# ViacheslavDanilov/oct_segmentation

Measured on AMD Instinct MI355X. Metric: OCT frames/sec (704x704, bf16) fwd+bwd, higher is better.
Workload: dtype bf16; 1 GPU; unetplusplus/resnet101 1-class 704x704, batch 16/GPU, fwd+Dice+bwd+allreduce+Adam; global_batch=16, parallelism=dp1

## Files before the change

oct_segmentation_amd/csrc/wgrad_mfma.hip:

```cpp
#include "common.h"
#include "conv_common.h"
#include "kernels.h"

#include <cstdlib>
#include <type_traits>

namespace octseg {

#ifdef OCTSEG_STAMP
#define WSTAMP(var) do { __builtin_amdgcn_sched_barrier(0); asm volatile("s_memtime %0\n\ts_waitcnt lgkmcnt(0)" : "=s"(var) :: "memory"); __builtin_amdgcn_sched_barrier(0); } while (0)
#else
#define WSTAMP(var) do { } while (0)
#endif

typedef __attribute__((ext_vector_type(4))) short s16x4_t;
typedef __attribute__((address_space(3))) s16x4_t lds_s16x4_t;

template <int NTAPS> struct WgradCfg { static constexpr int MAXW = NTAPS == 1 ? 4 : (NTAPS == 4 ? 6 : 7); };

__host__ __device__ constexpr int wrow_slots_before(int wr, int ks, int th) {
  int n = 0;
  for (int w = 0; w < wr; ++w) {
    const int klo = w - (ks - 1) < 0 ? 0 : w - (ks - 1), khi = w < th ? w : th - 1;
    n += (khi - klo + 1) * ks;
  }
  return n;
}

template <typename T, int NTAPS>
__global__ __launch_bounds__(NTHR) void wgrad_mfma_kernel(const WgradArgs a, const int th, const int pipelined) {
  extern __shared__ __attribute__((aligned(16))) char smem[];
  constexpr int VEC = Tr<T>::VEC;
  constexpr int RB = 64 * (int)sizeof(T);
  constexpr int PITCH = sizeof(T) == 2 ? 192 : RB + 16;
  constexpr int VPR = RB / 16;
  constexpr int PSTEP = NTHR / VPR;
  constexpr int MAXY = 4, MAXW = WgradCfg<NTAPS>::MAXW;
  typedef WindowStager<T, RB, NTHR, PITCH> Stager;

  const int tid = threadIdx.x, lane = tid & 63, wave = tid >> 6;
  const int wq_m = wave >> 1, wq_n = wave & 1;
  int bx = blockIdx.x, by = blockIdx.y, bz = blockIdx.z;
  {
    const int gx_ = gridDim.x, gy_ = gridDim.y, gz_ = gridDim.z;
    const int total = gx_ * gy_ * gz_;
    const int groups = gx_ * gz_;
    const int lid = bx + gx_ * (by + gy_ * bz);
    if (a.co_fast && (groups & 7) == 0) {
      const int x = lid & 7, q = lid >> 3;
      const int k = q / gy_, r = q - k * gy_;
      const int g = x * (groups >> 3) + k;
      by = r; bz = g / gx_; bx = g - bz * gx_;
    } else if (!a.co_fast && (total & 7) == 0 && (gz_ & 7) == 0) {
      const int w = (lid & 7) * (total >> 3) + (lid >> 3);
      bz = w / (gx_ * gy_);
      const int rem = w - bz * (gx_ * gy_);
      by = rem / gx_; bx = rem - by * gx_;
    }
  }
  const int ci0 = bx * 64, co0 = by * 64;

  const int tiles_x = (a.OW + TW - 1) / TW, tiles_y = (a.OH + th - 1) / th;
  const int ntiles = a.N * tiles_x * tiles_y;

  const bool single = a.ntaps == 1;
  const int lstride = single ? 1 : a.istride;
  const int smul = single ? a.istride : 1;
  const int RH = single ? th : (th - 1) * a.istride + a.span_y;
  const int RW = single ? TW : (TW - 1) * a.istride + a.span_x;
  const int npix = RH * RW;
  const int npw = (npix + PSTEP - 1) / PSTEP;
  const int npy = (th * TW + PSTEP - 1) / PSTEP;
  const float inv_rw = 1.0f / (float)RW;

  char* ldsY = smem;
  char* ldsX = smem + npy * PSTEP * PITCH;

  f32x16_t acc[NTAPS];
#pragma unroll
  for (int t = 0; t < NTAPS; ++t)
#pragma unroll
    for (int k = 0; k < 16; ++k) acc[t][k] = 0.f;

  int toff[NTAPS];
#pragma unroll
  for (int t = 0; t < NTAPS; ++t)
    toff[t] = single ? 0 : ((a.tap_dy[t] - a.min_dy) * RW + (a.tap_dx[t] - a.min_dx)) * PITCH;

  int ya0, xa0, xrow_step;
  if constexpr (sizeof(T) == 2) {
    const int g = lane >> 4, i = lane & 15, q = i >> 2, p = i & 3, hh = g >> 1, cb = g & 1;
    const int tx = 8 * hh + q;
    ya0 = tx * PITCH + (wq_m * 32 + 16 * cb + 4 * p) * 2;
    xa0 = (tx * lstride) * PITCH + (wq_n * 32 + 16 * cb + 4 * p) * 2;
    xrow_step = 4 * lstride * PITCH;
  } else {
    const int r = lane & 31, h = lane >> 5;
    ya0 = h * PITCH + (wq_m * 32 + r) * 4;
    xa0 = (h * lstride) * PITCH + (wq_n * 32 + r) * 4;
    xrow_step = 2 * lstride * PITCH;
  }

  Stager sg;
  sg.setup(a.src, a.nsrc, a.Cin, bx, tid);
  const int ycv = tid % VPR, yp0 = tid / VPR;
  const int yc = co0 + ycv * VEC;
  const bool ycok = yc < a.dyC;

  struct TilePos { int n, y0, x0; };
  auto tile_pos = [&](int tile) {
    TilePos tp;
    tp.n = tile / (tiles_x * tiles_y);
    const int rem = tile - tp.n * tiles_x * tiles_y;
    const int tyi = rem / tiles_x;
    tp.y0 = tyi * th; tp.x0 = (rem - tyi * tiles_x) * TW;
    return tp;
  };
  const int dy_pix_bytes = a.dyC * (int)sizeof(T), dy_row_bytes = a.DW * dy_pix_bytes;
  auto load_y = [&](const char* ybase, const TilePos& tp, int ty, int tx, bool in_tile, bool& ok) {
    const int gy = tp.y0 + ty, gx = tp.x0 + tx;
    ok = ycok && in_tile && gy < a.OH && gx < a.OW;
    const int gyc = min(gy, a.OH - 1), gxc = min(gx, a.OW - 1);
    const unsigned off = (unsigned)((gyc * a.dstride + a.doy) * dy_row_bytes + (gxc * a.dstride + a.dox) * dy_pix_bytes);
    return *(const uint4*)(ybase + off);
  };
  auto write_y = [&](int pass, uint4 v, bool ok) {
    *(uint4*)(ldsY + (pass * PSTEP + yp0) * PITCH + ycv * 16) = ok ? v : make_uint4(0, 0, 0, 0);
  };
  auto y_base = [&](int n) { return (const char*)a.dy + ((size_t)n * a.DH * a.DW * a.dyC + (ycok ? yc : 0)) * sizeof(T); };
  auto compute = [&]() {
    if constexpr (sizeof(T) == 2) {
      struct Pair { s16x4_t lo, hi; };
      struct Frags { uint4 y; uint4 x[NTAPS]; };
      auto load_frags = [&](int kk, Frags& f) {
        const char* yrow = ldsY + kk * TW * PITCH + ya0;
        const char* xrow = ldsX + (kk * lstride) * RW * PITCH + xa0;
        Pair ya;
        ya.lo = __builtin_amdgcn_ds_read_tr16_b64_v4i16((lds_s16x4_t*)(yrow));
        ya.hi = __builtin_amdgcn_ds_read_tr16_b64_v4i16((lds_s16x4_t*)(yrow + 4 * PITCH));
        f.y = __builtin_bit_cast(uint4, ya);
#pragma unroll
        for (int t = 0; t < NTAPS; ++t) {
          Pair xb;
          xb.lo = __builtin_amdgcn_ds_read_tr16_b64_v4i16((lds_s16x4_t*)(xrow + toff[t]));
          xb.hi = __builtin_amdgcn_ds_read_tr16_b64_v4i16((lds_s16x4_t*)(xrow + toff[t] + xrow_step));
          f.x[t] = __builtin_bit_cast(uint4, xb);
        }
      };
      auto load_y1 = [&](int kk, Frags& f) {
        const char* yrow = ldsY + kk * TW * PITCH + ya0;
        Pair ya;
        ya.lo = __builtin_amdgcn_ds_read_tr16_b64_v4i16((lds_s16x4_t*)(yrow));
        ya.hi = __builtin_amdgcn_ds_read_tr16_b64_v4i16((lds_s16x4_t*)(yrow + 4 * PITCH));
        f.y = __builtin_bit_cast(uint4, ya);
      };
      auto load_x1 = [&](const char* xrow, int t, Frags& f) {
        Pair xb;
        xb.lo = __builtin_amdgcn_ds_read_tr16_b64_v4i16((lds_s16x4_t*)(xrow + toff[t]));
        xb.hi = __builtin_amdgcn_ds_read_tr16_b64_v4i16((lds_s16x4_t*)(xrow + toff[t] + xrow_step));
        f.x[t] = __builtin_bit_cast(uint4, xb);
      };
      auto row_step = [&](const Frags& cur, int kn, Frags& nxt) {
        const char* xrow = ldsX + (kn * lstride) * RW * PITCH + xa0;
#pragma unroll
        for (int t = 0; t < NTAPS; ++t) {
          Tr<T>::mma(cur.y, cur.x[t], acc[t]);
          __builtin_amdgcn_sched_barrier(0);
          if (t == 0) load_y1(kn, nxt);
          load_x1(xrow, t, nxt);
          __builtin_amdgcn_sched_barrier(0);
        }
      };
      Frags fa, fb;
      load_frags(0, fa);
      for (int kk = 0; kk < th; kk += 2) {
        row_step(fa, min(kk + 1, th - 1), fb);
        if (kk + 1 < th) row_step(fb, min(kk + 2, th - 1), fa);
      }
    } else {
      for (int kk = 0; kk < th; ++kk) {
        const char* yrow = ldsY + kk * TW * PITCH + ya0;
        const char* xrow = ldsX + (kk * lstride) * RW * PITCH + xa0;
#pragma unroll
        for (int kp = 0; kp < 8; ++kp) {
          const float yv = *(const float*)(yrow + kp * 2 * PITCH);
#pragma unroll
          for (int t = 0; t < NTAPS; ++t) {
            const float xv = *(const float*)(xrow + toff[t] + kp * xrow_step);
            acc[t] = __builtin_amdgcn_mfma_f32_32x32x2f32(yv, xv, acc[t], 0, 0, 0);
          }
        }
      }
    }
  };

#ifdef OCTSEG_STAMP
  unsigned long long wts[5] = {0, 0, 0, 0, 0};
#endif
  if (pipelined) {
    uint4 yv[MAXY], xv[MAXW];
    bool yok[MAXY], xok[MAXW];
    int ypos[MAXY], wpos[MAXW];
    bool yin[MAXY], win[MAXW];
#pragma unroll
    for (int u = 0; u < MAXY; ++u) {
      const int p = min(u, npy - 1) * PSTEP + yp0;
      ypos[u] = ((p >> 4) << 16) | (p & 15);
      yin[u] = p < th * TW;
    }
#pragma unroll
    for (int u = 0; u < MAXW; ++u) {
      const int hp = min(u, npw - 1) * PSTEP + sg.p0;
      const int hy = (int)(((float)hp + 0.5f) * inv_rw);
      wpos[u] = (hy << 16) | (hp - hy * RW);
      win[u] = hp < npix;
    }
    auto load_tile = [&](int tile) {
      const TilePos tp = tile_pos(tile);
      const char* yb = y_base(tp.n);
      sg.bind_image(tp.n);
      const int gy0 = tp.y0 * a.istride + a.min_dy, gx0 = tp.x0 * a.istride + a.min_dx;
#pragma unroll
      for (int u = 0; u < MAXY; ++u) yv[u] = load_y(yb, tp, ypos[u] >> 16, ypos[u] & 0xffff, yin[u], yok[u]);
#pragma unroll
      for (int u = 0; u < MAXW; ++u)
        xv[u] = sg.load_at(wpos[u] >> 16, wpos[u] & 0xffff, win[u], gy0, gx0, smul, a.IH, a.IW, xok[u]);
    };
    auto write_tile = [&]() {
#pragma unroll
      for (int u = 0; u < MAXY; ++u) write_y(min(u, npy - 1), yv[u], yok[u]);
#pragma unroll
      for (int u = 0; u < MAXW; ++u) sg.write(ldsX, min(u, npw - 1), xv[u], xok[u]);
    };
    int tile = bz;
    if constexpr (sizeof(T) == 2 && (NTAPS == 9 || NTAPS == 4)) {
      if (pipelined == 2 && tile < ntiles) {
        constexpr int TH8 = 8, NSLOT = TH8 * NTAPS, NITEM = MAXY + MAXW, KS = NTAPS == 9 ? 3 : 2, RWC = TW + KS - 1, NWR = TH8 + KS - 1;
        const int tile_bytes = (npy + npw) * PSTEP * PITCH;
        TilePos tp2{0, 0, 0};
        const char* yb2 = nullptr;
        int gy02 = 0, gx02 = 0;
        auto item = [&](auto jc, auto phase, char* oy, char* ox) __attribute__((always_inline)) {
          constexpr int J = decltype(jc)::value;
          constexpr int PH = decltype(phase)::value;
          if constexpr (PH == 0) {
            if constexpr (J < MAXY) *(uint4*)(oy + (min(J, npy - 1) * PSTEP + yp0) * PITCH + ycv * 16) = yok[J] ? yv[J] : make_uint4(0, 0, 0, 0);
            else sg.write(ox, min(J - MAXY, npw - 1), xv[J - MAXY], xok[J - MAXY]);
          } else {
            if constexpr (J < MAXY) yv[J] = load_y(yb2, tp2, ypos[J] >> 16, ypos[J] & 0xffff, yin[J], yok[J]);
            else xv[J - MAXY] = sg.load_at(wpos[J - MAXY] >> 16, wpos[J - MAXY] & 0xffff, win[J - MAXY], gy02, gx02, smul, a.IH, a.IW, xok[J - MAXY]);
          }
        };
        auto fillers = [&](auto sc_, char* oy, char* ox) __attribute__((always_inline)) {
          constexpr int S = decltype(sc_)::value;
          constexpr int HALF = NSLOT / 2;
          constexpr int PH = S < HALF ? 0 : 1;
          constexpr int SS = S - PH * HALF;
          constexpr int J0 = (SS * NITEM + HALF - 1) / HALF, J1 = ((SS + 1) * NITEM + HALF - 1) / HALF;
          if constexpr (J0 < J1 && J0 < NITEM) item(std::integral_constant<int, J0>{}, std::integral_constant<int, PH>{}, oy, ox);
          if constexpr (J0 + 1 < J1 && J0 + 1 < NITEM) item(std::integral_constant<int, J0 + 1>{}, std::integral_constant<int, PH>{}, oy, ox);
          if constexpr (J0 + 2 < J1 && J0 + 2 < NITEM) item(std::integral_constant<int, J0 + 2>{}, std::integral_constant<int, PH>{}, oy, ox);
        };
        struct Frag { s16x4_t lo, hi; };
        Frag xs[2][KS], ys[4];
        auto rd_x = [&](const char* xbase, auto wc, auto sc, auto hc) __attribute__((always_inline)) {
          constexpr int Wn = decltype(wc)::value, S_ = decltype(sc)::value, H_ = decltype(hc)::value;
          constexpr int OFF = (Wn * RWC + S_) * PITCH + H_ * 4 * PITCH;
          if constexpr (H_ == 0) xs[Wn & 1][S_].lo = __builtin_amdgcn_ds_read_tr16_b64_v4i16((lds_s16x4_t*)(xbase + OFF));
          else xs[Wn & 1][S_].hi = __builtin_amdgcn_ds_read_tr16_b64_v4i16((lds_s16x4_t*)(xbase + OFF));
        };
        auto rd_y = [&](const char* ybase, auto kc, auto hc) __attribute__((always_inline)) {
          constexpr int Kn = decltype(kc)::value, H_ = decltype(hc)::value;
          constexpr int OFF = Kn * TW * PITCH + H_ * 4 * PITCH;
          if constexpr (H_ == 0) ys[Kn & 3].lo = __builtin_amdgcn_ds_read_tr16_b64_v4i16((lds_s16x4_t*)(ybase + OFF));
          else ys[Kn & 3].hi = __builtin_amdgcn_ds_read_tr16_b64_v4i16((lds_s16x4_t*)(ybase + OFF));
        };
        auto prefetch = [&](auto wc, auto qc, const char* xbase, const char* ybase) __attribute__((always_inline)) {
          constexpr int Q = decltype(qc)::value;
          if constexpr (Q < 2 * KS) rd_x(xbase, wc, std::integral_constant<int, Q / 2>{}, std::integral_constant<int, Q % 2>{});
          else rd_y(ybase, wc, std::integral_constant<int, Q - 2 * KS>{});
        };
        auto wrow = [&](auto wc, const char* by, const char* bx, char* oy, char* ox) __attribute__((always_inline)) {
          constexpr int Wr = decltype(wc)::value;
          constexpr int KLO = Wr - (KS - 1) < 0 ? 0 : Wr - (KS - 1), KHI = Wr < TH8 ? Wr : TH8 - 1;
          constexpr int CNT = (KHI - KLO + 1) * KS;
          constexpr int S0 = wrow_slots_before(Wr, KS, TH8);
          constexpr int NR = Wr + 1 >= NWR ? 0 : (Wr + 1 < TH8 ? 2 * KS + 2 : 2 * KS);
          const char* xbase = bx + xa0;
          const char* ybase = by + ya0;
          auto one = [&](auto jc) __attribute__((always_inline)) {
            constexpr int j = decltype(jc)::value;
            if constexpr (j < CNT) {
              constexpr int kk = KLO + j / KS, sft = j % KS, t = NTAPS == 9 ? (Wr - kk) * 3 + sft : (1 - (Wr - kk)) * 2 + (1 - sft);
              Tr<T>::mma(__builtin_bit_cast(uint4, ys[kk & 3]), __builtin_bit_cast(uint4, xs[Wr & 1][sft]), acc[t]);
              __builtin_amdgcn_sched_barrier(0);
              constexpr int R0 = j * NR / CNT, R1 = (j + 1) * NR / CNT;
              if constexpr (R0 < R1) prefetch(std::integral_constant<int, Wr + 1>{}, std::integral_constant<int, R0>{}, xbase, ybase);
              if constexpr (R0 + 1 < R1) prefetch(std::integral_constant<int, Wr + 1>{}, std::integral_constant<int, R0 + 1>{}, xbase, ybase);
              if constexpr (R0 + 2 < R1) prefetch(std::integral_constant<int, Wr + 1>{}, std::integral_constant<int, R0 + 2>{}, xbase, ybase);
              fillers(std::integral_constant<int, S0 + j>{}, oy, ox);
              __builtin_amdgcn_sched_barrier(0);
            }
          };
          one(std::integral_constant<int, 0>{}); one(std::integral_constant<int, 1>{}); one(std::integral_constant<int, 2>{});
          one(std::integral_constant<int, 3>{}); one(std::integral_constant<int, 4>{}); one(std::integral_constant<int, 5>{});
          one(std::integral_constant<int, 6>{}); one(std::integral_constant<int, 7>{}); one(std::integral_constant<int, 8>{});
        };
        load_tile(tile);
        write_tile();
        load_tile(tile + a.ksplit < ntiles ? tile + a.ksplit : tile);
        __syncthreads();
        int cur = 0;
        for (; tile < ntiles; tile += a.ksplit) {
          const int t2 = tile + 2 * a.ksplit < ntiles ? tile + 2 * a.ksplit : tile;
          tp2 = tile_pos(t2);
          yb2 = y_base(tp2.n);
          gy02 = tp2.y0 * a.istride + a.min_dy; gx02 = tp2.x0 * a.istride + a.min_dx;
          const char* by = smem + cur * tile_bytes;
          const char* bx = by + npy * PSTEP * PITCH;
          char* oy = smem + (cur ^ 1) * tile_bytes;
          char* ox = oy + npy * PSTEP * PITCH;
          {
            auto z = std::integral_constant<int, 0>{};
            auto o = std::integral_constant<int, 1>{};
            rd_y(by + ya0, z, z); rd_y(by + ya0, z, o);
            rd_x(bx + xa0, z, z, z); rd_x(bx + xa0, z, z, o);
            rd_x(bx + xa0, z, o, z); rd_x(bx + xa0, z, o, o);
            if constexpr (KS == 3) { rd_x(bx + xa0, z, std::integral_constant<int, 2>{}, z); rd_x(bx + xa0, z, std::integral_constant<int, 2>{}, o); }
          }
          wrow(std::integral_constant<int, 0>{}, by, bx, oy, ox);
          wrow(std::integral_constant<int, 1>{}, by, bx, oy, ox);
          wrow(std::integral_constant<int, 2>{}, by, bx, oy, ox);
          wrow(std::integral_constant<int, 3>{}, by, bx, oy, ox);
          if constexpr (KS == 2) sg.bind_image(tp2.n);
          wrow(std::integral_constant<int, 4>{}, by, bx, oy, ox);
          if constexpr (KS == 3) sg.bind_image(tp2.n);
          wrow(std::integral_constant<int, 5>{}, by, bx, oy, ox);
          wrow(std::integral_constant<int, 6>{}, by, bx, oy, ox);
          wrow(std::integral_constant<int, 7>{}, by, bx, oy, ox);
          wrow(std::integral_constant<int, 8>{}, by, bx, oy, ox);
          if constexpr (NWR > 9) wrow(std::integral_constant<int, 9>{}, by, bx, oy, ox);
          __builtin_amdgcn_sched_barrier(0);
          __syncthreads();
          cur ^= 1;
        }
        tile = ntiles;
      }
    }
    if (tile < ntiles) {
      load_tile(tile);
      write_tile();
      __syncthreads();
      for (; tile < ntiles; tile += a.ksplit) {
        unsigned long long w0 = 0, w1 = 0, w2 = 0, w3 = 0, w4 = 0; (void)w0; (void)w1; (void)w2; (void)w3; (void)w4;
        WSTAMP(w0);
        const int nxt = tile + a.ksplit < ntiles ? tile + a.ksplit : tile;
        load_tile(nxt);
        WSTAMP(w1);
        compute();
        WSTAMP(w2);
        __builtin_amdgcn_sched_barrier(0);
        __syncthreads();
        WSTAMP(w3);
        write_tile();
        __syncthreads();
        WSTAMP(w4);
#ifdef OCTSEG_STAMP
        wts[0] += w1 - w0; wts[1] += w2 - w1; wts[2] += w3 - w2; wts[3] += w4 - w3; wts[4] += 1;
#endif
      }
    }
  } else {
    for (int tile = bz; tile < ntiles; tile += a.ksplit) {
      const TilePos tp = tile_pos(tile);
      __syncthreads();
      for (int p = 0; p < npy; p += MAXY) {
        uint4 v[MAXY]; bool ok[MAXY];
#pragma unroll
        for (int u = 0; u < MAXY; ++u) {
          const int pp = min(p + u, npy - 1) * PSTEP + yp0;
          v[u] = load_y(y_base(tp.n), tp, pp >> 4, pp & 15, pp < th * TW, ok[u]);
        }
#pragma unroll
        for (int u = 0; u < MAXY; ++u) write_y(min(p + u, npy - 1), v[u], ok[u]);
      }
      for (int p = 0; p < npw; p += 4) {
        uint4 v[4]; bool ok[4];
#pragma unroll
        for (int u = 0; u < 4; ++u)
          v[u] = sg.load(min(p + u, npw - 1), tp.n, tp.y0 * a.istride + a.min_dy, tp.x0 * a.istride + a.min_dx, smul, RW,
                         npix, inv_rw, a.IH, a.IW, ok[u]);
#pragma unroll
        for (int u = 0; u < 4; ++u) sg.write(ldsX, min(p + u, npw - 1), v[u], ok[u]);
      }
      __syncthreads();
      compute();
    }
  }

#ifdef OCTSEG_STAMP
  if (a.stamp != nullptr && lane == 0)
    for (int i = 0; i < 5; ++i) atomicAdd(a.stamp + i, wts[i]);
#endif
  const int ci = ci0 + wq_n * 32 + (lane & 31);
#pragma unroll
  for (int t = 0; t < NTAPS; ++t) {
    const int tw = a.tap_w[t];
#pragma unroll
    for (int i = 0; i < 16; ++i) {
      const int co = co0 + wq_m * 32 + (i & 3) + 8 * (i >> 2) + 4 * (lane >> 5);
      if (co < a.Cout && ci < a.Cin) atomicAdd(a.dW + ((size_t)tw * a.Cout + co) * a.Cin + ci, acc[t][i]);
    }
  }
}

struct WgradGeom { int npy, npw; size_t lds; };
static WgradGeom wgrad_geom(const WgradArgs& a, int dtype, int th) {
  const int RB = 64 * (int)dtype_size(dtype), PITCH = dtype_size(dtype) == 2 ? 192 : RB + 16, PSTEP = NTHR / (RB / 16);
  const bool single = a.ntaps == 1;
  const int RH = single ? th : (th - 1) * a.istride + a.span_y;
  const int RW = single ? TW : (TW - 1) * a.istride + a.span_x;
  WgradGeom g;
  g.npy = (th * TW + PSTEP - 1) / PSTEP;
  g.npw = (RH * RW + PSTEP - 1) / PSTEP;
  g.lds = (size_t)(g.npy + g.npw) * PSTEP * PITCH;
  return g;
}

template <typename T, int NTAPS>
static hipError_t launch_wgrad_t(const WgradArgs& a0, int dtype, hipStream_t st) {
  WgradArgs a = a0;
  int th = 0, pipelined = 0;
  for (int cand = 8; cand >= 2; cand >>= 1) {
    const WgradGeom g = wgrad_geom(a, dtype, cand);
    if (g.npy <= 4 && g.npw <= WgradCfg<NTAPS>::MAXW && g.lds <= 150 * 1024) { th = cand; pipelined = 1; break; }
  }
  if (!th) {
    th = 8;
    while (th > 1 && wgrad_geom(a, dtype, th).lds > 150 * 1024) th >>= 1;
  }
  size_t lds = wgrad_geom(a, dtype, th).lds;
  bool std33 = NTAPS == 9 && a.istride == 1 && a.span_x == 3 && a.span_y == 3;
  for (int t = 0; std33 && t < 9; ++t) std33 = a.tap_dy[t] - a.min_dy == t / 3 && a.tap_dx[t] - a.min_dx == t % 3;
  bool std22 = NTAPS == 4 && a.istride == 1 && a.span_x == 2 && a.span_y == 2;
  for (int t = 0; std22 && t < 4; ++t) std22 = a.tap_dy[t] - a.min_dy == 1 - t / 2 && a.tap_dx[t] - a.min_dx == 1 - t % 2;
  if (pipelined && th == 8 && dtype != DT_F32 && (std33 || std22) && 2 * lds <= 150 * 1024) { pipelined = 2; lds *= 2; }
  const int ntiles = a.N * ((a.OW + TW - 1) / TW) * ((a.OH + th - 1) / th);
  const int gx = (a.Cin + 63) / 64, gy = (a.Cout + 63) / 64;
  const int wg_target = NTAPS == 1 ? 512 : (a.wg_target > 0 ? a.wg_target : 256);
  int ks = wg_target / (gx * gy);
  if (ks > ntiles) ks = ntiles;
  if (ks < 1) ks = 1;
  if (deterministic_mode()) ks = 1;
  a.ksplit = ks;
  static const bool ci_major = getenv("OCTSEG_WGRAD_CI_MAJOR") != nullptr;
  a.co_fast = ci_major ? 0 : 1;
  static bool attr_set = false;
  if (!attr_set) {
    hipError_t e = hipFuncSetAttribute((const void*)wgrad_mfma_kernel<T, NTAPS>,
                                       hipFuncAttributeMaxDynamicSharedMemorySize, 160 * 1024);
    if (e != hipSuccess) return e;
    attr_set = true;
  }
  hipLaunchKernelGGL((wgrad_mfma_kernel<T, NTAPS>), dim3(gx, gy, ks), dim3(NTHR), lds, st, a, th, pipelined);
  return hipGetLastError();
}

static void flatten_1x1(WgradArgs& a) {
  if (a.ntaps != 1 || a.istride != 1 || a.dstride != 1 || a.tap_dy[0] != 0 || a.tap_dx[0] != 0) return;
  const long long npix = (long long)a.N * a.OH * a.OW;
  if (npix % TW != 0 || a.IH != a.OH || a.IW != a.OW || a.DH != a.OH || a.DW != a.OW) return;
  for (int i = 0; i < a.nsrc; ++i)
    if (a.src[i].up || a.src[i].H != a.IH || a.src[i].W != a.IW) return;
  const int rows = (int)(npix / TW);
  a.N = 1; a.IH = a.OH = a.DH = rows; a.IW = a.OW = a.DW = TW;
  for (int i = 0; i < a.nsrc; ++i) { a.src[i].H = rows; a.src[i].W = TW; }
}

WgradRoute wgrad_route(const WgradArgs& a0, int dtype) {
  if (thin_wgrad_eligible(a0, dtype)) return WROUTE_THIN;
  WgradArgs a = a0;
  flatten_1x1(a);
  return wgrad1x1_eligible(a, dtype) ? WROUTE_1X1 : WROUTE_MFMA;
}

hipError_t launch_wgrad(int dtype, const WgradArgs& a0, hipStream_t st) {
  if (dtype == DT_F16) return hipErrorInvalidValue;

  if (a0.ntaps <= 0) return hipSuccess;
  const WgradRoute route = wgrad_route(a0, dtype);
  if (route == WROUTE_THIN) return launch_thin_wgrad(dtype, a0, st);
  WgradArgs a = a0;
  flatten_1x1(a);
  if (route == WROUTE_1X1) return launch_wgrad1x1(dtype, a, st);
  if (a.ntaps == 1 || a.ntaps == 4 || a.ntaps == 9) {
    if (dtype == DT_F32) {
      if (a.ntaps == 1) return launch_wgrad_t<float, 1>(a, dtype, st);
      if (a.ntaps == 4) return launch_wgrad_t<float, 4>(a, dtype, st);
      return launch_wgrad_t<float, 9>(a, dtype, st);
    }
    if (a.ntaps == 1) return launch_wgrad_t<bf16_t, 1>(a, dtype, st);
    if (a.ntaps == 4) return launch_wgrad_t<bf16_t, 4>(a, dtype, st);
    return launch_wgrad_t<bf16_t, 9>(a, dtype, st);
  }
  for (int t = 0; t < a.ntaps; ++t) {
    WgradArgs b = a;
    b.ntaps = 1;
    b.tap_dy[0] = a.tap_dy[t]; b.tap_dx[0] = a.tap_dx[t]; b.tap_w[0] = a.tap_w[t];
    b.min_dy = a.tap_dy[t]; b.min_dx = a.tap_dx[t]; b.span_y = 1; b.span_x = 1;
    hipError_t e = dtype == DT_F32 ? launch_wgrad_t<float, 1>(b, dtype, st) : launch_wgrad_t<bf16_t, 1>(b, dtype, st);
    if (e != hipSuccess) return e;
  }
  return hipSuccess;
}

}
```

Baseline: 257.6 frames/s.

## Add 16x16x32 MFMA variant of bf16 3x3 weight-gradient kernel with pair-row pipelining

Adds an MM=16 specialization of the wgrad kernel for bf16 standard 3x3 convolutions that uses 16x16 MFMA tiles with four accumulators per tap instead of one 32x32 accumulator. It uses a new LDS pitch (160), a new fragment addressing scheme, a pair-row step schedule interleaving LDS transposed reads and prefetch fillers, and a shuffle-based epilogue. The specialization is compiled in a separate translation unit and is routed to whenever the double-buffered std33 path would run. The intent is better MFMA throughput or scheduling and lower LDS use. The cost is more accumulators and register pressure, plus extra epilogue shuffles and atomics.

```diff
diff --git a/oct_segmentation_amd/csrc/wgrad_mfma.hip b/oct_segmentation_amd/csrc/wgrad_mfma.hip
--- a/oct_segmentation_amd/csrc/wgrad_mfma.hip
+++ b/oct_segmentation_amd/csrc/wgrad_mfma.hip
@@ -4,6 +4,7 @@
 
 #include <cstdlib>
 #include <type_traits>
+#include <utility>
 
 namespace octseg {
 
@@ -27,15 +28,24 @@
   return n;
 }
 
-template <typename T, int NTAPS>
+template <class F, int... I>
+__device__ __forceinline__ void static_for_seq(F&& f, std::integer_sequence<int, I...>) { (f(std::integral_constant<int, I>{}), ...); }
+template <int N, class F>
+__device__ __forceinline__ void static_for(F&& f) { static_for_seq(f, std::make_integer_sequence<int, N>{}); }
+
+__host__ __device__ constexpr int wgrad_pitch(int esize, int mm) { return esize == 2 ? (mm == 16 ? 160 : 192) : 64 * esize + 16; }
+
+template <typename T, int NTAPS, int MM = 32>
 __global__ __launch_bounds__(NTHR) void wgrad_mfma_kernel(const WgradArgs a, const int th, const int pipelined) {
   extern __shared__ __attribute__((aligned(16))) char smem[];
+  constexpr bool M16 = MM == 16;
+  static_assert(!M16 || (sizeof(T) == 2 && NTAPS == 9), "the 16x16x32 form exists for the bf16 3x3 loop");
   constexpr int VEC = Tr<T>::VEC;
   constexpr int RB = 64 * (int)sizeof(T);
-  constexpr int PITCH = sizeof(T) == 2 ? 192 : RB + 16;
+  constexpr int PITCH = wgrad_pitch((int)sizeof(T), MM);
   constexpr int VPR = RB / 16;
   constexpr int PSTEP = NTHR / VPR;
-  constexpr int MAXY = 4, MAXW = WgradCfg<NTAPS>::MAXW;
+  constexpr int MAXY = 4, MAXW = M16 ? 6 : WgradCfg<NTAPS>::MAXW;
   typedef WindowStager<T, RB, NTHR, PITCH> Stager;
 
   const int tid = threadIdx.x, lane = tid & 63, wave = tid >> 6;
@@ -76,11 +86,12 @@
   char* ldsY = smem;
   char* ldsX = smem + npy * PSTEP * PITCH;
 
-  f32x16_t acc[NTAPS];
-#pragma unroll
-  for (int t = 0; t < NTAPS; ++t)
-#pragma unroll
-    for (int k = 0; k < 16; ++k) acc[t][k] = 0.f;
+  constexpr int NACC = M16 ? 4 * NTAPS : NTAPS, ACCN = M16 ? 4 : 16;
+  typename std::conditional<M16, f32x4_t, f32x16_t>::type acc[NACC];
+#pragma unroll
+  for (int t = 0; t < NACC; ++t)
+#pragma unroll
+    for (int k = 0; k < ACCN; ++k) acc[t][k] = 0.f;
 
   int toff[NTAPS];
 #pragma unroll
@@ -88,7 +99,12 @@
     toff[t] = single ? 0 : ((a.tap_dy[t] - a.min_dy) * RW + (a.tap_dx[t] - a.min_dx)) * PITCH;
 
   int ya0, xa0, xrow_step;
-  if constexpr (sizeof(T) == 2) {
+  if constexpr (M16) {
+    const int g = lane >> 4, i = lane & 15, q = i >> 2, p = i & 3, px = 4 * (g & 1) + q;
+    ya0 = ((g >> 1) * 4 * TW + px) * PITCH + (wq_m * 32 + 4 * p) * 2;
+    xa0 = ((g >> 1) * 4 * (TW + 2) + px) * PITCH + (wq_n * 32 + 4 * p) * 2;
+    xrow_step = 0;
+  } else if constexpr (sizeof(T) == 2) {
     const int g = lane >> 4, i = lane & 15, q = i >> 2, p = i & 3, hh = g >> 1, cb = g & 1;
     const int tx = 8 * hh + q;
     ya0 = tx * PITCH + (wq_m * 32 + 16 * cb + 4 * p) * 2;
@@ -129,7 +145,8 @@
   };
   auto y_base = [&](int n) { return (const char*)a.dy + ((size_t)n * a.DH * a.DW * a.dyC + (ycok ? yc : 0)) * sizeof(T); };
   auto compute = [&]() {
-    if constexpr (sizeof(T) == 2) {
+    if constexpr (M16) {
+    } else if constexpr (sizeof(T) == 2) {
       struct Pair { s16x4_t lo, hi; };
       struct Frags { uint4 y; uint4 x[NTAPS]; };
       auto load_frags = [&](int kk, Frags& f) {
@@ -197,7 +214,7 @@
 #ifdef OCTSEG_STAMP
   unsigned long long wts[5] = {0, 0, 0, 0, 0};
 #endif
-  if (pipelined) {
+  if (M16 || pipelined) {
     uint4 yv[MAXY], xv[MAXW];
     bool yok[MAXY], xok[MAXW];
     int ypos[MAXY], wpos[MAXW];
@@ -234,8 +251,8 @@
     };
     int tile = bz;
     if constexpr (sizeof(T) == 2 && (NTAPS == 9 || NTAPS == 4)) {
-      if (pipelined == 2 && tile < ntiles) {
-        constexpr int TH8 = 8, NSLOT = TH8 * NTAPS, NITEM = MAXY + MAXW, KS = NTAPS == 9 ? 3 : 2, RWC = TW + KS - 1, NWR = TH8 + KS - 1;
+      if ((M16 || pipelined == 2) && tile < ntiles) {
+        constexpr int TH8 = 8, NSLOT = (M16 ? 2 : 1) * TH8 * NTAPS, NITEM = MAXY + MAXW, KS = NTAPS == 9 ? 3 : 2, RWC = TW + KS - 1, NWR = TH8 + KS - 1;
         const int tile_bytes = (npy + npw) * PSTEP * PITCH;
         TilePos tp2{0, 0, 0};
         const char* yb2 = nullptr;
@@ -292,7 +309,7 @@
             constexpr int j = decltype(jc)::value;
             if constexpr (j < CNT) {
               constexpr int kk = KLO + j / KS, sft = j % KS, t = NTAPS == 9 ? (Wr - kk) * 3 + sft : (1 - (Wr - kk)) * 2 + (1 - sft);
-              Tr<T>::mma(__builtin_bit_cast(uint4, ys[kk & 3]), __builtin_bit_cast(uint4, xs[Wr & 1][sft]), acc[t]);
+              if constexpr (!M16) Tr<T>::mma(__builtin_bit_cast(uint4, ys[kk & 3]), __builtin_bit_cast(uint4, xs[Wr & 1][sft]), acc[t]);
               __builtin_amdgcn_sched_barrier(0);
               constexpr int R0 = j * NR / CNT, R1 = (j + 1) * NR / CNT;
               if constexpr (R0 < R1) prefetch(std::integral_constant<int, Wr + 1>{}, std::integral_constant<int, R0>{}, xbase, ybase);
@@ -305,6 +322,40 @@
           one(std::integral_constant<int, 0>{}); one(std::integral_constant<int, 1>{}); one(std::integral_constant<int, 2>{});
           one(std::integral_constant<int, 3>{}); one(std::integral_constant<int, 4>{}); one(std::integral_constant<int, 5>{});
           one(std::integral_constant<int, 6>{}); one(std::integral_constant<int, 7>{}); one(std::integral_constant<int, 8>{});
+        };
+        constexpr int NPR = TH8 / 2, NWP = NPR + KS - 1, NSTEP = NWP * KS;
+        Frag xs16[3][2], ys16[3][2];
+        auto rd_x16 = [&](const char* xbase, auto nc, auto qc) __attribute__((always_inline)) {
+          constexpr int Nn = decltype(nc)::value, Q = decltype(qc)::value, Wn = Nn / KS, S_ = Nn % KS, B_ = Q / 2, H_ = Q % 2;
+          constexpr int OFF = (Wn * RWC + S_) * PITCH + H_ * 8 * PITCH + B_ * 32;
+          if constexpr (H_ == 0) xs16[Nn % 3][B_].lo = __builtin_amdgcn_ds_read_tr16_b64_v4i16((lds_s16x4_t*)(xbase + OFF));
+          else xs16[Nn % 3][B_].hi = __builtin_amdgcn_ds_read_tr16_b64_v4i16((lds_s16x4_t*)(xbase + OFF));
+        };
+        auto rd_y16 = [&](const char* ybase, auto kc, auto qc) __attribute__((always_inline)) {
+          constexpr int Kn = decltype(kc)::value, Q = decltype(qc)::value, B_ = Q / 2, H_ = Q % 2;
+          constexpr int OFF = Kn * TW * PITCH + H_ * 8 * PITCH + B_ * 32;
+          if constexpr (H_ == 0) ys16[Kn % 3][B_].lo = __builtin_amdgcn_ds_read_tr16_b64_v4i16((lds_s16x4_t*)(ybase + OFF));
+          else ys16[Kn % 3][B_].hi = __builtin_amdgcn_ds_read_tr16_b64_v4i16((lds_s16x4_t*)(ybase + OFF));
+        };
+        auto step16 = [&](auto nc, const char* by, const char* bx, char* oy, char* ox) __attribute__((always_inline)) {
+          constexpr int Nn = decltype(nc)::value, Wr = Nn / KS, sft = Nn % KS;
+          constexpr int KLO = Wr - (KS - 1) < 0 ? 0 : Wr - (KS - 1), KHI = Wr < NPR ? Wr : NPR - 1;
+          constexpr int CNT = (KHI - KLO + 1) * 4;
+          constexpr int S0 = wrow_slots_before(Wr, KS, NPR) * 4 + sft * CNT;
+          constexpr int YJ0 = (Wr + 1 < KS && sft == 0) ? 0 : ((Wr + 1 >= KS && Wr + 1 < NPR && sft == KS - 1) ? 4 : -1);
+          const char* xbase = bx + xa0;
+          const char* ybase = by + ya0;
+          static_for<CNT>([&](auto jc) __attribute__((always_inline)) {
+            constexpr int j = decltype(jc)::value;
+            constexpr int kk = KLO + j / 4, cb = (j >> 1) & 1, ib = j & 1, t = (Wr - kk) * 3 + sft;
+            if constexpr (M16)
+              Tr<T>::mma16(__builtin_bit_cast(uint4, ys16[kk % 3][cb]), __builtin_bit_cast(uint4, xs16[Nn % 3][ib]), acc[(t * 2 + cb) * 2 + ib]);
+            __builtin_amdgcn_sched_barrier(0);
+            if constexpr (j < 4 && Nn + 2 < NSTEP) rd_x16(xbase, std::integral_constant<int, Nn + 2>{}, jc);
+            if constexpr (YJ0 >= 0 && j >= YJ0 && j < YJ0 + 4) rd_y16(ybase, std::integral_constant<int, Wr + 1>{}, std::integral_constant<int, j - YJ0>{});
+            fillers(std::integral_constant<int, S0 + j>{}, oy, ox);
+            __builtin_amdgcn_sched_barrier(0);
+          });
         };
         load_tile(tile);
         write_tile();
@@ -320,7 +371,18 @@
           const char* bx = by + npy * PSTEP * PITCH;
           char* oy = smem + (cur ^ 1) * tile_bytes;
           char* ox = oy + npy * PSTEP * PITCH;
-          {
+          if constexpr (M16) {
+            auto z = std::integral_constant<int, 0>{};
+            auto o = std::integral_constant<int, 1>{};
+            rd_y16(by + ya0, z, z); rd_y16(by + ya0, z, o);
+            rd_x16(bx + xa0, z, z); rd_x16(bx + xa0, z, o);
+            static_for<2>([&](auto qc) __attribute__((always_inline)) { rd_y16(by + ya0, z, std::integral_constant<int, 2 + decltype(qc)::value>{}); });
+            static_for<2>([&](auto qc) __attribute__((always_inline)) { rd_x16(bx + xa0, z, std::integral_constant<int, 2 + decltype(qc)::value>{}); });
+            static_for<4>([&](auto qc) __attribute__((always_inline)) { rd_x16(bx + xa0, o, qc); });
+            static_for<9>([&](auto nc) __attribute__((always_inline)) { step16(nc, by, bx, oy, ox); });
+            sg.bind_image(tp2.n);
+            static_for<9>([&](auto nc) __attribute__((always_inline)) { step16(std::integral_constant<int, 9 + decltype(nc)::value>{}, by, bx, oy, ox); });
+          } else {
             auto z = std::integral_constant<int, 0>{};
             auto o = std::integral_constant<int, 1>{};
             rd_y(by + ya0, z, z); rd_y(by + ya0, z, o);
@@ -328,18 +390,20 @@
             rd_x(bx + xa0, z, o, z); rd_x(bx + xa0, z, o, o);
             if constexpr (KS == 3) { rd_x(bx + xa0, z, std::integral_constant<int, 2>{}, z); rd_x(bx + xa0, z, std::integral_constant<int, 2>{}, o); }
           }
-          wrow(std::integral_constant<int, 0>{}, by, bx, oy, ox);
-          wrow(std::integral_constant<int, 1>{}, by, bx, oy, ox);
-          wrow(std::integral_constant<int, 2>{}, by, bx, oy, ox);
-          wrow(std::integral_constant<int, 3>{}, by, bx, oy, ox);
-          if constexpr (KS == 2) sg.bind_image(tp2.n);
-          wrow(std::integral_constant<int, 4>{}, by, bx, oy, ox);
-          if constexpr (KS == 3) sg.bind_image(tp2.n);
-          wrow(std::integral_constant<int, 5>{}, by, bx, oy, ox);
-          wrow(std::integral_constant<int, 6>{}, by, bx, oy, ox);
-          wrow(std::integral_constant<int, 7>{}, by, bx, oy, ox);
-          wrow(std::integral_constant<int, 8>{}, by, bx, oy, ox);
-          if constexpr (NWR > 9) wrow(std::integral_constant<int, 9>{}, by, bx, oy, ox);
+          if constexpr (!M16) {
+            wrow(std::integral_constant<int, 0>{}, by, bx, oy, ox);
+            wrow(std::integral_constant<int, 1>{}, by, bx, oy, ox);
+            wrow(std::integral_constant<int, 2>{}, by, bx, oy, ox);
+            wrow(std::integral_constant<int, 3>{}, by, bx, oy, ox);
+            if constexpr (KS == 2) sg.bind_image(tp2.n);
+            wrow(std::integral_constant<int, 4>{}, by, bx, oy, ox);
+            if constexpr (KS == 3) sg.bind_image(tp2.n);
+            wrow(std::integral_constant<int, 5>{}, by, bx, oy, ox);
+            wrow(std::integral_constant<int, 6>{}, by, bx, oy, ox);
+            wrow(std::integral_constant<int, 7>{}, by, bx, oy, ox);
+            wrow(std::integral_constant<int, 8>{}, by, bx, oy, ox);
+            if constexpr (NWR > 9) wrow(std::integral_constant<int, 9>{}, by, bx, oy, ox);
+          }
           __builtin_amdgcn_sched_barrier(0);
           __syncthreads();
           cur ^= 1;
@@ -347,7 +411,7 @@
         tile = ntiles;
       }
     }
-    if (tile < ntiles) {
+    if (!M16 && tile < ntiles) {
       load_tile(tile);
       write_tile();
       __syncthreads();
@@ -403,20 +467,40 @@
     for (int i = 0; i < 5; ++i) atomicAdd(a.stamp + i, wts[i]);
 #endif
   const int ci = ci0 + wq_n * 32 + (lane & 31);
-#pragma unroll
-  for (int t = 0; t < NTAPS; ++t) {
-    const int tw = a.tap_w[t];
-#pragma unroll
-    for (int i = 0; i < 16; ++i) {
-      const int co = co0 + wq_m * 32 + (i & 3) + 8 * (i >> 2) + 4 * (lane >> 5);
-      if (co < a.Cout && ci < a.Cin) atomicAdd(a.dW + ((size_t)tw * a.Cout + co) * a.Cin + ci, acc[t][i]);
+  if constexpr (M16) {
+    const bool odd = (lane >> 4) & 1;
+    const int corow = co0 + wq_m * 32 + 8 * (lane >> 5);
+#pragma unroll
+    for (int t = 0; t < NTAPS; ++t) {
+      const int tw = a.tap_w[t];
+#pragma unroll
+      for (int cb = 0; cb < 2; ++cb)
+#pragma unroll
+        for (int r = 0; r < 4; ++r) {
+          const float l = acc[(t * 2 + cb) * 2][r], rt = acc[(t * 2 + cb) * 2 + 1][r];
+          const float got = __shfl_xor(odd ? l : rt, 16);
+          const float v0 = odd ? got : l, v1 = odd ? rt : got;
+          const int co = corow + 16 * cb + r;
+          if (co < a.Cout && ci < a.Cin) atomicAdd(a.dW + ((size_t)tw * a.Cout + co) * a.Cin + ci, v0);
+          if (co + 4 < a.Cout && ci < a.Cin) atomicAdd(a.dW + ((size_t)tw * a.Cout + co + 4) * a.Cin + ci, v1);
+        }
+    }
+  } else {
+#pragma unroll
+    for (int t = 0; t < NTAPS; ++t) {
+      const int tw = a.tap_w[t];
+#pragma unroll
+      for (int i = 0; i < 16; ++i) {
+        const int co = co0 + wq_m * 32 + (i & 3) + 8 * (i >> 2) + 4 * (lane >> 5);
+        if (co < a.Cout && ci < a.Cin) atomicAdd(a.dW + ((size_t)tw * a.Cout + co) * a.Cin + ci, acc[t][i]);
+      }
     }
   }
 }
 
 struct WgradGeom { int npy, npw; size_t lds; };
-static WgradGeom wgrad_geom(const WgradArgs& a, int dtype, int th) {
-  const int RB = 64 * (int)dtype_size(dtype), PITCH = dtype_size(dtype) == 2 ? 192 : RB + 16, PSTEP = NTHR / (RB / 16);
+static WgradGeom wgrad_geom(const WgradArgs& a, int dtype, int th, int mm = 32) {
+  const int RB = 64 * (int)dtype_size(dtype), PITCH = wgrad_pitch((int)dtype_size(dtype), mm), PSTEP = NTHR / (RB / 16);
   const bool single = a.ntaps == 1;
   const int RH = single ? th : (th - 1) * a.istride + a.span_y;
   const int RW = single ? TW : (TW - 1) * a.istride + a.span_x;
@@ -426,6 +510,26 @@
   g.lds = (size_t)(g.npy + g.npw) * PSTEP * PITCH;
   return g;
 }
+
+template <typename T, int NTAPS, int MM>
+static hipError_t launch_wgrad_kernel(const WgradArgs& a, dim3 grid, size_t lds, int th, int pipelined, hipStream_t st) {
+  static bool attr_set = false;
+  if (!attr_set) {
+    hipError_t e = hipFuncSetAttribute((const void*)wgrad_mfma_kernel<T, NTAPS, MM>,
+                                       hipFuncAttributeMaxDynamicSharedMemorySize, 160 * 1024);
+    if (e != hipSuccess) return e;
+    attr_set = true;
+  }
+  hipLaunchKernelGGL((wgrad_mfma_kernel<T, NTAPS, MM>), grid, dim3(NTHR), lds, st, a, th, pipelined);
+  return hipGetLastError();
+}
+
+hipError_t launch_wgrad_m16(const WgradArgs& a, dim3 grid, size_t lds, int th, hipStream_t st);
+#ifdef OCTSEG_WGRAD_M16_TU
+hipError_t launch_wgrad_m16(const WgradArgs& a, dim3 grid, size_t lds, int th, hipStream_t st) {
+  return launch_wgrad_kernel<bf16_t, 9, 16>(a, grid, lds, th, 2, st);
+}
+#else
 
 template <typename T, int NTAPS>
 static hipError_t launch_wgrad_t(const WgradArgs& a0, int dtype, hipStream_t st) {
@@ -455,15 +559,10 @@
   a.ksplit = ks;
   static const bool ci_major = getenv("OCTSEG_WGRAD_CI_MAJOR") != nullptr;
   a.co_fast = ci_major ? 0 : 1;
-  static bool attr_set = false;
-  if (!attr_set) {
-    hipError_t e = hipFuncSetAttribute((const void*)wgrad_mfma_kernel<T, NTAPS>,
-                                       hipFuncAttributeMaxDynamicSharedMemorySize, 160 * 1024);
-    if (e != hipSuccess) return e;
-    attr_set = true;
-  }
-  hipLaunchKernelGGL((wgrad_mfma_kernel<T, NTAPS>), dim3(gx, gy, ks), dim3(NTHR), lds, st, a, th, pipelined);
-  return hipGetLastError();
+  if constexpr (sizeof(T) == 2 && NTAPS == 9) {
+    if (pipelined == 2 && std33) return launch_wgrad_m16(a, dim3(gx, gy, ks), 2 * wgrad_geom(a, dtype, th, 16).lds, th, st);
+  }
+  return launch_wgrad_kernel<T, NTAPS, 32>(a, dim3(gx, gy, ks), lds, th, pipelined, st);
 }
 
 static void flatten_1x1(WgradArgs& a) {
@@ -513,5 +612,6 @@
   }
   return hipSuccess;
 }
-
-}
+#endif
+
+}
diff --git a/oct_segmentation_amd/csrc/wgrad_mfma_m16.hip b/oct_segmentation_amd/csrc/wgrad_mfma_m16.hip
--- /dev/null
+++ b/oct_segmentation_amd/csrc/wgrad_mfma_m16.hip
@@ -0,0 +1,2 @@
+#define OCTSEG_WGRAD_M16_TU
+#include "wgrad_mfma.hip"
```

Result: no change. 259.3 frames/s, median of 6 (+0.7%).
